# martinber/noaa-apt

Measured on AMD Instinct MI355X. Metric: Msamples/sec WAV->APT-line decode, higher is better.
Workload: dtype f32; 1 GPU; synthetic 48000 Hz APT recording, 600 s (28800000 samples) per GPU, profile=standard: resample 13/50 (959 taps) -> AM envelope -> 37-tap low-pass -> sync correlation + peak picker -> 1198 rows x 2080 px; parallelism=1 GPU(s), 16 independent recordings per GPU and step, no collectives, recordings_per_call=16, mode=strict, rows=1198, n_sync=1199, input_resident_in_hbm=True, distinct_inputs_round_robin=16

## Files before the change

### noaa_apt_amd/csrc/apt_capi.hip

```cpp
#include <cstdio>
#include <cstdlib>
#include <cstring>
#include <memory>
#include <string>

#include "apt_capi_util.hpp"
#include "apt_session.hpp"

namespace {

using namespace apt::capi;

using PlanPtr = std::unique_ptr<aptgpu_plan, apt::capi::PlanDeleter>;


apt::Signal download(const float *d, size_t n, hipStream_t s)
{
    apt::Signal h(n);
    if (n) {
        apt::hip_check(hipMemcpyAsync(h.data(), d, n * sizeof(float), hipMemcpyDeviceToHost, s),
                       "hipMemcpyAsync D2H");
        apt::hip_check(hipStreamSynchronize(s), "hipStreamSynchronize");
    }
    return h;
// ... 66 lines not shown
int aptgpu_plan_get_info(const aptgpu_plan *plan, aptgpu_plan_info *info)
{
    if (!plan || !info) return APTGPU_ERR_INVALID;
    info->l = plan->l;
    info->m = plan->m;
    info->n_resample_taps = static_cast<uint32_t>(plan->taps_resample.size());
    info->n_lowpass_taps = static_cast<uint32_t>(plan->taps_lowpass.size());
    info->n_sync_taps = plan->n_sync_taps;
    info->samples_per_work_row = plan->spr;
    info->min_distance = plan->md;
    info->max_samples = plan->max_samples;
    info->max_work_len = plan->max_work_len;
    info->max_rows = plan->max_rows;
    info->fused = plan->fused;
    info->max_batch = plan->max_batch;
    return APTGPU_OK;
}

int aptgpu_plan_decode_device(aptgpu_plan *plan, int count, const float *const *d_signals,
                              const size_t *n, float *const *d_rows, const size_t *rows_cap,
                              char *err, size_t err_cap)
{
    if (!plan || !d_signals || !n || !d_rows || !rows_cap || count < 0 ||
        count > plan->max_batch) {
        put_err(err, err_cap, "bad argument to aptgpu_plan_decode_device");
        return APTGPU_ERR_INVALID;
    }
    return guarded(err, err_cap, [&] {
        apt::hip_check(hipSetDevice(plan->device), "hipSetDevice");
        for (int i = 0; i < count; ++i)
            if (n[i] > plan->max_samples)
                throw Error{ErrorKind::Invalid, "recording longer than the plan's max_samples"};
        std::vector<aptgpu_plan::Input> ins(static_cast<size_t>(count));
        std::vector<uint64_t> caps(static_cast<size_t>(count));
        for (int i = 0; i < count; ++i) {
            ins[static_cast<size_t>(i)].ptr = d_signals[i];
            ins[static_cast<size_t>(i)].n = n[i];
            caps[static_cast<size_t>(i)] = static_cast<uint64_t>(rows_cap[i]) * 2080u;
        }
        plan->run_call(count, ins.data(), d_rows, caps.data(), false);
        return APTGPU_OK;
    });
}

int aptgpu_plan_synchronize(aptgpu_plan *plan)
{
    if (!plan) return APTGPU_ERR_INVALID;
    (void)hipSetDevice(plan->device);
    try {
        plan->sync_all();
    } catch (const Error &) {
        return APTGPU_ERR_HIP;
    }
    return APTGPU_OK;
}

int aptgpu_plan_join(aptgpu_plan *plan)
{
    if (!plan) return APTGPU_ERR_INVALID;
    if (!plan->user_stream) return aptgpu_plan_synchronize(plan);
    (void)hipSetDevice(plan->device);
    for (hipStream_t st : plan->streams) {
        if (hipEventRecord(plan->ev_user, st) != hipSuccess ||
            hipStreamWaitEvent(plan->user_stream, plan->ev_user, 0) != hipSuccess)
            return APTGPU_ERR_HIP;
    }
    return APTGPU_OK;
}

int aptgpu_plan_results(aptgpu_plan *plan, int count, aptgpu_result *results)
{
    if (!plan || !results || count < 0 || static_cast<size_t>(count) > plan->last_slots.size())
        return APTGPU_ERR_INVALID;
    static_assert(sizeof(aptgpu_result) == sizeof(apt::gpu::Result), "result layout");
    (void)hipSetDevice(plan->device);
    try {
        plan->sync_all();
    } catch (const Error &) {
        return APTGPU_ERR_HIP;
    }
    for (int i = 0; i < count; ++i)
        if (hipMemcpy(results + i, plan->result_of(i), sizeof(aptgpu_result), hipMemcpyDeviceToHost) !=
            hipSuccess)
            return APTGPU_ERR_HIP;
    return APTGPU_OK;
}

int aptgpu_plan_sync_positions(aptgpu_plan *plan, int i, uint64_t *pos, size_t cap, size_t *n_sync)
{
    if (!plan || i < 0 || static_cast<size_t>(i) >= plan->last_slots.size() || !n_sync)
        return APTGPU_ERR_INVALID;
    aptgpu_result r{};
    (void)hipSetDevice(plan->device);
    try {
        plan->sync_all();
    } catch (const Error &) {
        return APTGPU_ERR_HIP;
    }
    if (hipMemcpy(&r, plan->result_of(i), sizeof r, hipMemcpyDeviceToHost) != hipSuccess)
        return APTGPU_ERR_HIP;
    *n_sync = r.n_sync;
    size_t take = r.n_sync < cap ? r.n_sync : cap;
    if (!plan->sync || !pos || take == 0) return APTGPU_OK;
    if (take > plan->slot_of(i).peaks.count) take = plan->slot_of(i).peaks.count;
    std::vector<uint32_t> tmp(take);
    if (hipMemcpy(tmp.data(), plan->slot_of(i).peaks.ptr, take * sizeof(uint32_t),
                  hipMemcpyDeviceToHost) != hipSuccess)
        return APTGPU_ERR_HIP;
    for (size_t k = 0; k < take; ++k) pos[k] = tmp[k];
    return APTGPU_OK;
}

int aptgpu_plan_enable_timing(aptgpu_plan *plan, int on)
{
    if (!plan) return APTGPU_ERR_INVALID;
    plan->timer.enable(on < 0 ? 0 : (on > 2 ? 2 : on));
    return APTGPU_OK;
}

int aptgpu_plan_collect_timing(aptgpu_plan *plan, aptgpu_kernel_time *out, size_t cap, size_t *n_out)
{
    if (!plan || !n_out) return APTGPU_ERR_INVALID;
    try {
        (void)hipSetDevice(plan->device);
        plan->sync_all();
        plan->sync_all();
        auto v = plan->timer.collect(plan->stream);
        *n_out = v.size();
        for (size_t i = 0; i < v.size() && i < cap && out; ++i) out[i] = v[i];
        return APTGPU_OK;
    } catch (const Error &) {
        return APTGPU_ERR_HIP;
    }
}

int aptgpu_plan_read_internal(aptgpu_plan *plan, int i, const char *name, void *host_out,
                              size_t bytes, size_t *size_out)
{
    if (!plan || !name || i < 0 || static_cast<size_t>(i) >= plan->last_slots.size())
        return APTGPU_ERR_INVALID;
    aptgpu_plan::Slot &sl = plan->slot_of(i);
    const void *src = nullptr;
    size_t size = 0;
    const std::string n(name);
    if (n == "inv_sinphi") {
        if (size_out) *size_out = sizeof(float);
        if (host_out && bytes >= sizeof(float)) std::memcpy(host_out, &plan->inv_sinphi, sizeof(float));
        return APTGPU_OK;
    }
    if (n == "filtered") { src = sl.filtered.ptr; size = sl.filtered.count * sizeof(float); }
    else if (n == "correlation") { src = sl.correlation.ptr; size = sl.correlation.count * sizeof(float); }
    else if (n == "group_max") { src = sl.gm.ptr; size = sl.gm.count * sizeof(apt::gpu::GroupMax); }
    else if (n == "terminal_words") { src = sl.words.ptr; size = sl.words.count * sizeof(uint64_t); }
    else if (n == "peaks") { src = sl.peaks.ptr; size = sl.peaks.count * sizeof(uint32_t); }
    else if (n == "picker_flags") { src = sl.flags.ptr; size = sl.flags.count * sizeof(uint32_t); }
    else return APTGPU_ERR_INVALID;
    if (size_out) *size_out = size;
    (void)hipSetDevice(plan->device);
    try {
        plan->sync_all();
    } catch (const Error &) {
        return APTGPU_ERR_HIP;
    }
    const size_t take = bytes < size ? bytes : size;
    if (take && host_out && src &&
        hipMemcpy(host_out, src, take, hipMemcpyDeviceToHost) != hipSuccess)
        return APTGPU_ERR_HIP;
    return APTGPU_OK;
}

}

namespace apt::capi {

int decode_host(const aptgpu_context *ctx_in, const aptgpu_settings *settings, const float *signal,
                const uint8_t *wav_data, const apt::WavInfo *wav, size_t n, uint32_t input_rate_hz, int sync,
                float **rows_out, size_t *n_out, aptgpu_stats *stats, char *err, size_t err_cap)
{
    *rows_out = nullptr;
    *n_out = 0;
    aptgpu_context ctx = ctx_in ? *ctx_in : default_ctx();
    const bool steps = settings->export_wav != 0 && ctx.step != nullptr;

    return guarded(err, err_cap, [&]() -> int {
        const uint32_t work = settings->work_rate;
        if (!wav) step(&ctx, steps, "input", 0, signal, n, input_rate_hz);
        if (!wav || !steps) status(&ctx, 0.1f, "Resampling to " + std::to_string(work));

        const bool cached = !steps && ctx.stream == nullptr;
        SessionLease lease;
        struct PoisonOnThrow {
            SessionLease &l;
            bool ok = false;
            ~PoisonOnThrow() { if (!ok && l) l.poison(); }
        } guard{lease};
        hipStream_t s_for_errors = nullptr;
        auto decode_error = [&](const char *msg) -> Error {
            if (s_for_errors == nullptr || hipStreamSynchronize(s_for_errors) == hipSuccess) guard.ok = true;
            return Error{ErrorKind::Internal, msg};
        };
        PlanPtr own_plan;
        aptgpu_plan *plan = nullptr;
        if (cached) {
            SessionKey key;
            key.device = ctx.device;
            key.mode = ctx.mode;
            key.rate = input_rate_hz;
            key.sync = sync != 0;
            key.per_call = 1;
            key.settings = *settings;
            key.settings.export_wav = 0;
            key.settings.export_resample_filtered = settings->export_resample_filtered ? 1 : 0;
            lease = session_acquire(key, n);
            plan = lease->plan.get();
        } else {
            own_plan.reset(apt::plan_create(&ctx, *settings, input_rate_hz, sync != 0, n, 1,  1));
            plan = own_plan.get();
        }
        if (plan->spr == 0) throw Error{ErrorKind::Invalid, "work_rate too small"};
        hipStream_t s = plan->stream;
        s_for_errors = s;
        const uint64_t w = plan->work_len_for(n);
        const uint64_t out_cap =
            sync ? (plan->spr ? w / plan->spr + 2 : 2) * 2080u : plan->out_len_nosync(w) + 16;

        apt::DeviceBuffer<float> own_in, own_rows;
        apt::DeviceBuffer<uint8_t> own_wav;
        const size_t in_bytes = wav ? wav->data_len : n * sizeof(float);
        void *d_in_ptr = nullptr;
        float *d_rows_ptr = nullptr;
        if (cached) {
            lease->ensure_set(0, in_bytes + 64, out_cap);
            d_in_ptr = lease->sets[0].in[0].ptr;
            d_rows_ptr = lease->sets[0].out[0].ptr;
        } else if (wav) {
            own_wav.alloc(in_bytes + 16);
            d_in_ptr = own_wav.ptr;
        } else {
            own_in.alloc(n + 16);
            d_in_ptr = own_in.ptr;
        }
        if (!cached) {
            own_rows.alloc(out_cap);
            d_rows_ptr = own_rows.ptr;
        }
        struct { float *ptr; } d_rows{d_rows_ptr};
        aptgpu_plan::Input in;
        in.n = n;
        in.ptr = d_in_ptr;
        if (in_bytes)
            apt::hip_check(hipMemcpyAsync(d_in_ptr, wav ? static_cast<const void *>(wav_data) : static_cast<const void *>(signal),
                                          in_bytes, hipMemcpyHostToDevice, s), "hipMemcpyAsync H2D");
        if (wav) {
            in.channels = wav->channels;
            in.bytes_per_sample = wav->bytes_per_sample;
            in.codec = static_cast<int>(wav->codec);
        }

        float *rows_ptr = d_rows.ptr;
        const uint64_t cap64 = out_cap;
        plan->run_call(1, &in, &rows_ptr, &cap64, steps);
        aptgpu_plan::Slot &sl = plan->slot_of(0);
        if (steps) plan->sync_all();
        if (wav && steps) {
            apt::Signal x = download(sl.ingest.ptr, n, s);
            step(&ctx, steps, "input", 0, x.data(), x.size(), input_rate_hz);
            status(&ctx, 0.1f, "Resampling to " + std::to_string(work));
        }

        auto export_expanded = [&](uint64_t cnt, uint32_t rate, auto &&fill) {
            try {
                apt::DeviceBuffer<float> d_ex;
                d_ex.alloc(cnt + 16);
                fill(d_ex.ptr);
                apt::Signal ex = download(d_ex.ptr, cnt, s);
                step(&ctx, steps, "resample_filtered", 0, ex.data(), ex.size(), rate);
                return;
            } catch (const Error &e) {
                if (e.kind != ErrorKind::Hip || e.hip_code != static_cast<int>(hipErrorOutOfMemory)) throw;
                (void)hipGetLastError();
            } catch (const std::bad_alloc &) {
            }
            std::fprintf(stderr, "aptgpu: expanded filtered signal (%llu samples) can't fit in memory, skipping step\n",
                         static_cast<unsigned long long>(cnt));
            step(&ctx, steps, "resample_filtered", 0, nullptr, 0, rate);
        };
        step(&ctx, steps, "resample_filter", 1, plan->taps_resample.data(),
             plan->taps_resample.size(), 0);
        if (w < 10ull * plan->spr) throw decode_error(kTooShort);
        if (steps) {
            if (plan->l > 1 && plan->export_filtered) {
                const uint64_t cnt = apt::fast_resampling_export_geom(n, plan->l, plan->m, plan->taps_resample.size()).expanded;
                export_expanded(cnt, input_rate_hz * plan->l, [&](float *d_ex) {
                    plan->expanded_filtered(s, wav ? sl.ingest.ptr : static_cast<const float *>(d_in_ptr), n, false, d_ex, cnt);
                });
            } else if (plan->l > 1) {
                step(&ctx, steps, "resample_filtered", 0, nullptr, 0, input_rate_hz * plan->l);
            } else {
                apt::DeviceBuffer<float> d_fl;
                d_fl.alloc(n + 16);
                apt::gpu::fir_decimate(s, wav ? sl.ingest.ptr : static_cast<const float *>(d_in_ptr), n, plan->d_taps_resample.ptr,
                                       static_cast<uint32_t>(plan->taps_resample.size()), 1, d_fl.ptr, n);
                apt::Signal fl = download(d_fl.ptr, n, s);
                step(&ctx, steps, "resample_filtered", 0, fl.data(), fl.size(), input_rate_hz);
            }
            apt::Signal r = download(sl.resampled.ptr, w, s);
// ... 361 lines not shown
```

### noaa_apt_amd/csrc/apt_kernels_sync.hip

```cpp
#include "apt_kernels.hpp"
#include "apt_sync_corr.hpp"

#include <hip/hip_runtime.h>

#include <atomic>

#include <cstdlib>
#include <type_traits>

namespace apt::gpu {

namespace {

constexpr int GS = 52;
constexpr uint64_t kGroupMask = (1ull << GS) - 1;
constexpr float kNegInf = -__builtin_huge_valf();

__global__ void __launch_bounds__(256)
k_group_max(const float *__restrict__ corr, uint64_t n_corr, GroupMax *__restrict__ gm, uint32_t ng)
{
    const uint32_t g = blockIdx.x * blockDim.x + threadIdx.x;
    if (g >= ng) return;
    const uint64_t base = static_cast<uint64_t>(g) * GS;
    float mx = kNegInf;
    bool has_nan = false;
    for (int o = 0; o < GS; ++o) {
        const uint64_t i = base + o;
        if (i < n_corr) {
            float v = corr[i];
            if (i == 0 && !(v > 0.f)) v = 0.f;
            mx = fmaxf(mx, v);
            has_nan = has_nan || (v != v);
        }
    }
    gm[g] = has_nan ? GroupMax{-kNegInf, kNegInf} : GroupMax{mx, mx};
}

constexpr int kNodesThreads = 128;
constexpr int kNodesWaves = kNodesThreads / 64;
constexpr int kChunkGroups = 128;
constexpr int kSlotCap = 64;
static_assert(kNodesThreads == kChunkGroups, "one thread per own group");
constexpr uint32_t kNanStartTag = 0x80000000u;
constexpr uint32_t kPosMask = 0x7FFFFFFFu;

__host__ __device__ constexpr uint32_t nodes_window(uint32_t pw) { return (GS + 38u * pw - 1u + 3u) & ~3u; }

__device__ __forceinline__ float wave_prefix_max_dpp(float x)
{
    asm volatile("s_nop 1\n\tv_max_f32_dpp %0, %0, %0 row_shr:1 row_mask:0xf bank_mask:0xf\n\t"
                 "s_nop 1\n\tv_max_f32_dpp %0, %0, %0 row_shr:2 row_mask:0xf bank_mask:0xf\n\t"
                 "s_nop 1\n\tv_max_f32_dpp %0, %0, %0 row_shr:4 row_mask:0xf bank_mask:0xf\n\t"
                 "s_nop 1\n\tv_max_f32_dpp %0, %0, %0 row_shr:8 row_mask:0xf bank_mask:0xf\n\t"
                 "s_nop 1\n\tv_max_f32_dpp %0, %0, %0 row_bcast:15 row_mask:0xa bank_mask:0xf\n\t"
                 "s_nop 1\n\tv_max_f32_dpp %0, %0, %0 row_bcast:31 row_mask:0xc bank_mask:0xf\n\t"
                 "s_nop 1"
                 : "+v"(x));
    return x;
}
__device__ __forceinline__ float wave_suffix_max_excl_dpp(float x, int lane)
{
    float y = -__builtin_huge_valf();
    asm volatile("s_nop 1\n\tv_mov_b32_dpp %0, %1 wave_shl:1 row_mask:0xf bank_mask:0xf\n\t"
                 "s_nop 1\n\tv_max_f32_dpp %0, %0, %0 row_shl:1 row_mask:0xf bank_mask:0xf\n\t"
                 "s_nop 1\n\tv_max_f32_dpp %0, %0, %0 row_shl:2 row_mask:0xf bank_mask:0xf\n\t"
                 "s_nop 1\n\tv_max_f32_dpp %0, %0, %0 row_shl:4 row_mask:0xf bank_mask:0xf\n\t"
                 "s_nop 1\n\tv_max_f32_dpp %0, %0, %0 row_shl:8 row_mask:0xf bank_mask:0xf\n\t"
                 "s_nop 1"
                 : "+v"(y)
                 : "v"(x));
    const float r1 = __builtin_bit_cast(float, __builtin_amdgcn_readlane(__builtin_bit_cast(int, y), 16));
    const float r2 = __builtin_bit_cast(float, __builtin_amdgcn_readlane(__builtin_bit_cast(int, y), 32));
    const float r3 = __builtin_bit_cast(float, __builtin_amdgcn_readlane(__builtin_bit_cast(int, y), 48));
    const float m23 = fmaxf(r2, r3), m123 = fmaxf(r1, m23);
    const float tail = lane < 16 ? m123 : lane < 32 ? m23 : lane < 48 ? r3 : -__builtin_huge_valf();
    return fmaxf(y, tail);
}

__host__ __device__ constexpr uint32_t words_f32_ofs() { return kChunkGroups * 16u; }
__host__ __device__ constexpr uint32_t words_win_ofs(uint32_t r)
{
    return (words_f32_ofs() + (kChunkGroups + r + 1) * 16u + kChunkGroups * 4u + kChunkGroups * 2u + 15u) & ~15u;
}

template <int NL, int PWC>
__device__ __forceinline__ float nodes_eval_window(float *win, bool on, int lane, uint32_t pw, int fast)
{
    constexpr int NLR = NL > 0 ? NL : 1;
    float c = kNegInf;
    if (fast) {
        const uint32_t blen = GS + 36u * pw;
        if constexpr (NL > 0) {
            float bs[NLR];
#pragma unroll
            for (int t = 0; t < NL; ++t) {
                const uint32_t pq = lane + 64u * t;
                bs[t] = pq < blen ? sync_pulse_sum(pw, [&](uint32_t j) { return win[pq + j]; }) : 0.f;
            }
            __builtin_amdgcn_wave_barrier();
#pragma unroll
            for (int t = 0; t < NL; ++t) {
                const uint32_t pq = lane + 64u * t;
                if (pq < blen) win[pq] = bs[t];
            }
            __builtin_amdgcn_wave_barrier();
        } else {
            for (uint32_t p0 = 0; p0 < blen; p0 += 64) {
                const uint32_t pq = p0 + lane;
                const float bs = pq < blen ? sync_pulse_sum(pw, [&](uint32_t j) { return win[pq + j]; }) : 0.f;
                __builtin_amdgcn_wave_barrier();
                if (pq < blen) win[pq] = bs;
                __builtin_amdgcn_wave_barrier();
            }
        }
        if (on) c = sync_corr_from_pulses([&](int k) { return win[lane + k * 2 * pw]; });
    } else {
        if constexpr (PWC >= 4) {
            if (on) c = sync_corr_strict_rolled(pw, [&](uint32_t j) { return win[lane + j]; });
        } else {
            if (on) c = sync_corr_strict(pw, [&](uint32_t j) { return win[lane + j]; });
        }
    }
    return c;
}

template <int NL, int PWC, bool DPP>
__global__ void __launch_bounds__(kNodesThreads, 4)
k_sync_words(const CallArgs call, const SlotPtrs *__restrict__ slots, uint32_t pw_arg, uint32_t r_groups ,
             int fast, int use_corr)
{
    const uint32_t pw = PWC > 0 ? static_cast<uint32_t>(PWC) : pw_arg;
    const RecArgs rec = call.rec[blockIdx.y];
    const uint64_t w = rec.w;
    const uint64_t n_corr = w - 38ull * pw;
    const uint32_t ng = static_cast<uint32_t>((n_corr + GS - 1) / GS);
    if (blockIdx.x * static_cast<uint32_t>(kChunkGroups) >= ng) return;
    const SlotPtrs sp = slots[rec.slot];
    const GroupMax *__restrict__ gm = sp.gm;
    const float *__restrict__ corr = use_corr ? sp.corr : nullptr;
    const float *__restrict__ fsig = sp.f;
    uint32_t *__restrict__ flags = sp.flags;

    extern __shared__ uint64_t lds_nodes[];
    const int R = static_cast<int>(r_groups);
    const int N = kChunkGroups + R + 1;
    uint64_t *s_words = lds_nodes;
    uint64_t *s_nanw = s_words + kChunkGroups;
    float *s_hi = reinterpret_cast<float *>(reinterpret_cast<char *>(lds_nodes) + words_f32_ofs());
    float *s_lo = s_hi + N;
    float *s_ma = s_lo + N;
    float *s_mb = s_ma + N;
    float *s_wm = s_mb + N;
    uint16_t *s_cand = reinterpret_cast<uint16_t *>(s_wm + kChunkGroups);
    const uint32_t wlen = nodes_window(pw);
    float *s_win = reinterpret_cast<float *>(reinterpret_cast<char *>(lds_nodes) + words_win_ofs(r_groups));
    __shared__ uint32_t s_ncand;

    const int tid = threadIdx.x;
    const int lane = tid & 63;
    const int wave = tid >> 6;
    const int64_t g0 = static_cast<int64_t>(blockIdx.x) * kChunkGroups;
    const int64_t gw0 = g0;
    const uint64_t md = static_cast<uint64_t>(R) * GS;

    if (tid == 0) s_ncand = 0;
    if (blockIdx.x == 0 && tid == 0) {
        sp.res->status = -1;
        sp.res->reason = -1;
    }
    for (int q = tid; q < N; q += kNodesThreads) {
        const int64_t g = g0 + q;
        const GroupMax v = g < static_cast<int64_t>(ng) ? gm[g] : GroupMax{kNegInf, kNegInf};
        s_hi[q] = v.hi;
        s_lo[q] = v.lo;
        s_ma[q] = v.lo;
    }
    s_words[tid] = 0ull;
    s_nanw[tid] = 0ull;
    __syncthreads();

    {
        const int W = R - 1;
        float *a = s_ma, *bq = s_mb;
        int K = 1;
        for (; 2 * K <= W; K *= 2) {
            for (int q = tid; q < N; q += kNodesThreads) bq[q] = (q + K < N) ? fmaxf(a[q], a[q + K]) : a[q];
            __syncthreads();
            float *t = a; a = bq; bq = t;
        }
        const int q = tid;
        const int64_t g = g0 + q;
        const float wm = fmaxf(a[q + 1], a[q + 1 + W - K]);
        s_wm[q] = wm;
        if (g < static_cast<int64_t>(ng) && !(wm > s_hi[q])) s_cand[atomicAdd(&s_ncand, 1u)] = static_cast<uint16_t>(q);
        __syncthreads();
    }

    const uint32_t ncand = s_ncand;
    constexpr int kBatch = NL > 0 ? 4 : 1;
    constexpr int NLR = NL > 0 ? NL : 1;
    constexpr uint16_t kDeferred = 0x8000u;
    float *wa = s_win + static_cast<size_t>(wave) * wlen;
    const uint32_t wneed = GS + 38u * pw - 1u;
    auto eval_group = [&](uint64_t base, bool on) -> float {
        for (uint32_t t = lane; t < wlen; t += 64) {
            const uint64_t j = base + t;
            wa[t] = (t < wneed && j < w) ? fsig[j] : 0.f;
        }
        __builtin_amdgcn_wave_barrier();
        const float v = nodes_eval_window<NL, PWC>(wa, on, lane, pw, fast);
        __builtin_amdgcn_wave_barrier();
        return v;
    };
    auto settle = [&](auto exact_tag, int q, float cv, float c2v, bool in_v) -> bool {
        constexpr bool EXACT = decltype(exact_tag)::value;
        const uint64_t base = static_cast<uint64_t>(gw0 + q) * GS;
        const bool in2 = in_v && base + lane + md < n_corr;
        if (in_v && gw0 + q == 0 && lane == 0 && !(cv > 0.f)) cv = 0.f;
        const unsigned long long nanword = __ballot(in_v && cv != cv) & kGroupMask;
        if (cv != cv) cv = kNegInf;
        float sfx_ex;
        if constexpr (DPP) {
            sfx_ex = wave_suffix_max_excl_dpp(cv, lane);
        } else {
            float sfx = cv;
            for (int d = 1; d < 64; d <<= 1) {
                const float o = __shfl_down(sfx, d, 64);
                if (lane + d < 64) sfx = fmaxf(sfx, o);
            }
            sfx_ex = __shfl_down(sfx, 1, 64);
            if (lane == 63) sfx_ex = kNegInf;
        }
        float wm = s_wm[q];
        const bool open_lo = in_v && !(sfx_ex > cv) && !(wm > cv);
        if (__ballot(open_lo) != 0ull) {
            float wm_hi = kNegInf;
            for (int h = q + 1 + lane; h < q + R; h += 64) wm_hi = fmaxf(wm_hi, s_hi[h]);
            for (int d = 32; d >= 1; d >>= 1) wm_hi = fmaxf(wm_hi, __shfl_xor(wm_hi, d, 64));
            const bool open = open_lo && wm_hi > cv;
            if (__ballot(open) != 0ull) {
                if constexpr (!EXACT) {
                    return false;
                } else {
                    float thr = open ? cv : -kNegInf;
                    for (int d = 32; d >= 1; d >>= 1) thr = fminf(thr, __shfl_xor(thr, d, 64));
                    float ex = kNegInf;
#pragma unroll 1
                    for (int h0 = q + 1; h0 < q + R; h0 += 64) {
                        unsigned long long todo = __ballot(h0 + lane < q + R && s_hi[h0 + lane] > thr);
                        while (todo) {
                            const int h = h0 + __ffsll(static_cast<long long>(todo)) - 1;
                            todo &= todo - 1;
                            const int64_t gh = gw0 + h;
                            if (gh >= static_cast<int64_t>(ng)) break;
                            const uint64_t hb = static_cast<uint64_t>(gh) * GS;
                            const bool on = lane < GS && hb + lane < n_corr;
                            float v = kNegInf;
                            if (corr != nullptr) {
                                if (on) v = corr[hb + lane];
                            } else {
                                v = eval_group(hb, on);
                            }
                            if (v != v) v = kNegInf;
                            ex = fmaxf(ex, v);
                        }
                    }
                    for (int d = 32; d >= 1; d >>= 1) ex = fmaxf(ex, __shfl_xor(ex, d, 64));
                    if (open) wm = ex;
                    if (lane == 0) atomicAdd(&flags[7], 1u);
                }
            }
        }
        float wmax = fmaxf(sfx_ex, wm);
        const float gm_ahead = s_hi[q + R];
        if (corr == nullptr && __ballot(in2 && !(wmax > cv) && gm_ahead > cv) != 0ull) c2v = eval_group(base + md, in2);
        if (c2v != c2v) c2v = kNegInf;
        float pfx = c2v;
        if constexpr (DPP) {
            pfx = wave_prefix_max_dpp(pfx);
        } else {
            for (int d = 1; d < 64; d <<= 1) {
                const float o = __shfl_up(pfx, d, 64);
                if (lane >= d) pfx = fmaxf(pfx, o);
            }
        }
        wmax = fmaxf(wmax, pfx);
        const bool term = in_v && !(wmax > cv);
        const unsigned long long word = __ballot(term) & kGroupMask;
        if (lane == 0) {
            s_words[q] = word;
            s_nanw[q] = nanword;
        }
        __builtin_amdgcn_wave_barrier();
        return true;
    };
    bool any_deferred = false;
    for (uint32_t c0 = wave * kBatch; c0 < ncand; c0 += kBatch * kNodesWaves) {
        int qv[kBatch];
        float cv[kBatch], c2v[kBatch];
        bool inv[kBatch];
        float fa[kBatch][NLR];
#pragma unroll
        for (int e = 0; e < kBatch; ++e) {
            const uint32_t ci = c0 + e;
            qv[e] = (ci < ncand) ? s_cand[ci] : -1;
            const int64_t g = gw0 + (qv[e] < 0 ? 0 : qv[e]);
            const uint64_t i = static_cast<uint64_t>(g) * GS + lane;
            inv[e] = qv[e] >= 0 && lane < GS && i < n_corr;
            cv[e] = kNegInf;
            c2v[e] = kNegInf;
            if (corr != nullptr) {
                if (inv[e]) {
                    cv[e] = corr[i];
                    if (i + md < n_corr) c2v[e] = corr[i + md];
                }
            } else if constexpr (NL > 0) {
#pragma unroll
                for (int t = 0; t < NL; ++t) {
                    const uint64_t j = static_cast<uint64_t>(g) * GS + lane + 64u * t;
                    fa[e][t] = (qv[e] >= 0 && lane + 64u * t < wneed && j < w) ? fsig[j] : 0.f;
                }
            }
        }
#pragma unroll
        for (int e = 0; e < kBatch; ++e) {
            if (qv[e] < 0) continue;
            if (corr == nullptr) {
                if constexpr (NL > 0) {
#pragma unroll
                    for (int t = 0; t < NL; ++t)
                        if (lane + 64u * t < wlen) wa[lane + 64 * t] = fa[e][t];
                    __builtin_amdgcn_wave_barrier();
                    cv[e] = nodes_eval_window<NL, PWC>(wa, inv[e], lane, pw, fast);
                    __builtin_amdgcn_wave_barrier();
                } else {
                    cv[e] = eval_group(static_cast<uint64_t>(gw0 + qv[e]) * GS, inv[e]);
                }
            }
            if (!settle(std::false_type{}, qv[e], cv[e], c2v[e], inv[e])) {
                if (lane == 0) s_cand[c0 + e] = static_cast<uint16_t>(qv[e]) | kDeferred;
                any_deferred = true;
            }
        }
    }
    if (any_deferred) {
#pragma unroll 1
        for (uint32_t c0 = wave * kBatch; c0 < ncand; c0 += kBatch * kNodesWaves) {
#pragma unroll 1
            for (uint32_t ci = c0; ci < c0 + kBatch && ci < ncand; ++ci) {
                const uint16_t ent = s_cand[ci];
                if (!(ent & kDeferred)) continue;
                const int q = ent & (kDeferred - 1);
                const uint64_t base = static_cast<uint64_t>(gw0 + q) * GS;
                const bool in_v = lane < GS && base + lane < n_corr;
                float cv = kNegInf, c2v = kNegInf;
                if (corr != nullptr) {
                    if (in_v) {
                        cv = corr[base + lane];
                        if (base + lane + md < n_corr) c2v = corr[base + lane + md];
                    }
                } else {
                    cv = eval_group(base, in_v);
                }
                (void)settle(std::true_type{}, q, cv, c2v, in_v);
            }
        }
    }
    __syncthreads();

    {
        const int64_t g = g0 + tid;
        if (g < static_cast<int64_t>(ng)) {
            sp.words[g] = s_words[tid];
            sp.nanw[g] = s_nanw[tid];
        }
    }
}

__global__ void __launch_bounds__(kNodesThreads)
k_sync_slots(const CallArgs call, const SlotPtrs *__restrict__ slots, uint32_t pw, uint32_t r_groups ,
             uint32_t grid_groups )
{
    const RecArgs rec = call.rec[blockIdx.y];
    const uint64_t n_corr = rec.w - 38ull * pw;
    const uint32_t ng = static_cast<uint32_t>((n_corr + GS - 1) / GS);
    if (blockIdx.x * static_cast<uint32_t>(kChunkGroups) >= ng) return;
    const SlotPtrs sp = slots[rec.slot];
    const uint64_t *__restrict__ words = sp.words;
    const uint64_t *__restrict__ nanw = sp.nanw;
    uint32_t *__restrict__ slot_nt = sp.slot_nt;
    __shared__ uint32_t s_scan[kNodesWaves];
    const int tid = threadIdx.x;
    const int lane = tid & 63;
    const int wave = tid >> 6;
    const int64_t R = r_groups;
    const int64_t g = static_cast<int64_t>(blockIdx.x) * kChunkGroups + tid;
    auto word_at = [&](const uint64_t *p, int64_t gi) -> uint64_t {
        return (gi >= 0 && gi < static_cast<int64_t>(ng)) ? p[gi] : 0ull;
    };
    uint64_t nw = 0, ns = 0;
    if (g < static_cast<int64_t>(ng)) {
        const uint64_t wd = words[g];
        const uint64_t nb = nanw[g];
        const uint64_t prev_bit = word_at(words, g - 1) >> (GS - 1);
        const uint64_t heads = wd & ~(((wd << 1) | prev_bit) & kGroupMask);
        const uint64_t shifted = ((word_at(words, g - R) << 1) | (word_at(words, g - R - 1) >> (GS - 1))) & kGroupMask;
        const uint64_t shifted_nan = ((word_at(nanw, g - R) << 1) | (word_at(nanw, g - R - 1) >> (GS - 1))) & kGroupMask;
        const uint64_t on_grid = (g % grid_groups == 0) ? 1ull : 0ull;
        const uint64_t starts = shifted | shifted_nan | on_grid;
        nw = wd & (heads | starts);
        ns = nb & starts & ~wd;
    }
    const uint32_t cnt = static_cast<uint32_t>(__popcll(nw | ns));
    uint32_t inc = cnt;
    for (int d = 1; d < 64; d <<= 1) {
        const uint32_t o = __shfl_up(inc, d, 64);
        if (lane >= d) inc += o;
    }
    if (lane == 63) s_scan[wave] = inc;
    __syncthreads();
    uint32_t base = 0;
    for (int wv = 0; wv < wave; ++wv) base += s_scan[wv];
    uint32_t total = 0;
    for (int wv = 0; wv < kNodesWaves; ++wv) total += s_scan[wv];
    uint32_t ofs = base + inc - cnt;
    uint64_t bitsleft = nw | ns;
    while (bitsleft) {
        const int bpos = __ffsll(static_cast<long long>(bitsleft)) - 1;
        bitsleft &= bitsleft - 1;
        if (ofs < kSlotCap)
            slot_nt[static_cast<uint64_t>(blockIdx.x) * kSlotCap + ofs] =
                static_cast<uint32_t>(static_cast<uint64_t>(g) * GS + bpos) | (((ns >> bpos) & 1ull) ? kNanStartTag : 0u);
        ++ofs;
    }
    if (tid == 0) {
        sp.slot_cnt[blockIdx.x] = total;
        if (total > kSlotCap) atomicOr(&sp.flags[0], 1u);
    }
}

constexpr int kOrbitThreadsMax = 1024;
constexpr int kMaxLevels = 64;

struct OrbitGeom {
    uint64_t n_corr, work_len;
    uint32_t spr, md;
};

__device__ __forceinline__ uint64_t first_terminal52(const uint64_t *__restrict__ words,
                                                     uint64_t n_groups, uint64_t s)
{
    const int lane = threadIdx.x & 63;
    uint64_t g0 = s / GS;
    const uint32_t sh = static_cast<uint32_t>(s % GS);
    bool first = true;
    while (true) {
        const uint64_t gi = g0 + lane;
        uint64_t word = (gi < n_groups) ? words[gi] : 0ull;
        if (first && lane == 0) word &= (~0ull) << sh;
        const unsigned long long any = __ballot(word != 0ull);
        if (any) {
            const int src = __ffsll(static_cast<long long>(any)) - 1;
            const uint64_t pos = gi * GS + (__ffsll(static_cast<long long>(word)) - 1);
            return __shfl(pos, src, 64);
        }
        first = false;
        g0 += 64;
        if (g0 >= n_groups) return ~0ull;
    }
}

__device__ void orbit_walk52(const uint64_t *__restrict__ words, const uint64_t *__restrict__ nanw,
                             const OrbitGeom &gq, uint32_t *__restrict__ peaks, uint32_t peaks_cap,
                             Result *__restrict__ res)
{
    auto nan_at = [&](uint64_t s) -> bool { return (nanw[s / GS] >> (s % GS)) & 1ull; };
    const int lane = threadIdx.x & 63;
    const uint64_t n_groups = (gq.n_corr + GS - 1) / GS;
    const uint64_t spr = gq.spr, md = gq.md;
    uint64_t len = 1;
    uint64_t u = 0;
    if (gq.n_corr > 0) u = first_terminal52(words, n_groups, 0);
    if (lane == 0 && peaks_cap > 0) peaks[0] = static_cast<uint32_t>(u);
    uint64_t fit = (u + spr < gq.work_len) ? 1 : 0;
    uint64_t last_fit = fit;
    while (gq.n_corr > 0) {
        const uint64_t a = u + md + 1;
        const uint64_t b = (len + 1) * spr;
        const uint64_t s = a > b ? a : b;
        if (s >= gq.n_corr) break;
        const uint64_t c = s / spr;
        for (uint64_t q = len + lane; q + 1 < c; q += 64)
            if (q < peaks_cap) peaks[q] = static_cast<uint32_t>(s);
        if (s + spr < gq.work_len) fit += c - len - 1;
        u = nan_at(s) ? s : first_terminal52(words, n_groups, s);
        if (lane == 0 && c - 1 < peaks_cap) peaks[c - 1] = static_cast<uint32_t>(u);
        last_fit = (u + spr < gq.work_len) ? 1 : 0;
        fit += last_fit;
        len = c;
    }
    if (lane == 0) {
        const bool few = len < 5;
        res->status = few ? 1 : 0;
        res->reason = few ? 2 : 0;
        res->n_sync = static_cast<uint32_t>(len);
        res->n_rows = few ? 0 : static_cast<uint32_t>(fit - last_fit);
        res->work_len = gq.work_len;
        res->n_out = few ? 0 : (fit - last_fit) * 2080u;
    }
}


__device__ __forceinline__ uint32_t gld(const uint32_t *p)
{
    return __hip_atomic_load(p, __ATOMIC_RELAXED, __HIP_MEMORY_SCOPE_AGENT);
}
__device__ __forceinline__ void gst(uint32_t *p, uint32_t v)
{
    __hip_atomic_store(p, v, __ATOMIC_RELAXED, __HIP_MEMORY_SCOPE_AGENT);
}
template <int NT>
__global__ void __launch_bounds__(NT, NT >= 1024 ? 8 : 2)
k_sync_orbit_global(const CallArgs call, const SlotPtrs *__restrict__ slots, uint32_t spr_in, uint32_t md_in,
                    uint32_t pw, int force_walk, uint32_t lds_entries, int alg)
{
    const RecArgs rec = call.rec[blockIdx.x];
    const SlotPtrs sp = slots[rec.slot];
    const uint64_t *__restrict__ words = sp.words;
// ... 512 lines not shown
        if (tid == 0) {
            flags[1] = 1u;
            flags[0] = 0u;
            flags[5] = 0u;
            flags[11] = flags7;
            flags[7] = 0u;
        }
        return;
    }
    if (tid == 0 && !all_done) { gst(w_ja + END, END); gst(w_jb + END, END); gst(w_path, 0u); }
    __syncthreads();

    const uint32_t path_cap = kc + 2;
    const bool direct = !all_done && s_conflict == 0;
    if (direct) {
        const uint32_t endc = s_endcell;
        for (uint32_t k = tid + 1; k < path_cap; k += NT)
            gst(w_path + k, k < endc ? gld(w_succ + k) : END);
        __syncthreads();
    }
    uint32_t *ja = w_ja, *jb = w_jb;
    const uint32_t lds_cap = lds_entries;
    const bool in_lds = !all_done && !direct && path_cap + 2 * (count + 1) <= lds_cap && count < 0xFFFFu;
    if (in_lds) {
        uint16_t *pth = lds_orbit;
        uint16_t *la = pth + path_cap;
        uint16_t *lb = la + (count + 1);
        const uint16_t ENDC = static_cast<uint16_t>(count);
        for (uint32_t idx = tid; idx < count; idx += NT) {
            const uint32_t nx = gld(w_ja + gld(w_list + idx));
            la[idx] = nx == END ? ENDC : static_cast<uint16_t>(nx < base_d ? nx : gld(w_jb + nx));
        }
        if (tid == 0) { la[count] = ENDC; lb[count] = ENDC; pth[0] = 0; }
        __syncthreads();
        for (uint32_t span = 1; span < path_cap; span <<= 1) {
            for (uint32_t mI = tid; mI < span && mI + span < path_cap; mI += NT) pth[mI + span] = la[pth[mI]];
            for (uint32_t idx = tid; idx < count; idx += NT) lb[idx] = la[la[idx]];
            __syncthreads();
            uint16_t *t = la; la = lb; lb = t;
        }
        for (uint32_t k = tid; k < path_cap; k += NT)
            gst(w_path + k, pth[k] == ENDC ? END : gld(w_list + pth[k]));
        __syncthreads();
    }
    if (!all_done && !direct && !in_lds) {
    constexpr int kKeep = 4;
    uint32_t vk[kKeep], jk[kKeep];
#pragma unroll
    for (int j = 0; j < kKeep; ++j) {
        const uint32_t idx = tid + j * NT;
        vk[j] = (idx < count) ? gld(w_list + idx) : END;
    }
#pragma unroll
    for (int j = 0; j < kKeep; ++j) jk[j] = gld(ja + vk[j]);
    for (uint32_t span = 1; span < path_cap; span <<= 1) {
        for (uint32_t mI = tid; mI < span && mI + span < path_cap; mI += NT)
            gst(w_path + mI + span, gld(ja + gld(w_path + mI)));
#pragma unroll
        for (int j = 0; j < kKeep; ++j) jk[j] = gld(ja + jk[j]);
#pragma unroll
        for (int j = 0; j < kKeep; ++j) gst(jb + vk[j], jk[j]);
        for (uint32_t idx = tid + kKeep * NT; idx < count; idx += NT) {
            const uint32_t v = gld(w_list + idx);
            gst(jb + v, gld(ja + gld(ja + v)));
        }
        __syncthreads();
        uint32_t *t = ja; ja = jb; jb = t;
    }
    }
    if (!peaks_done) stamp(1);

    if (!peaks_done) {
    if (tid == 0) { s_plen = 1; s_fit = 0ull; }
    __syncthreads();
    }
    unsigned long long fit_local = 0;
    for (uint32_t k = tid; !peaks_done && k < path_cap; k += NT) {
        const uint32_t v = gld(w_path + k);
        if (v == END) continue;
        uint32_t cell;
        const uint32_t sv = node_start(v, &cell);
        const uint32_t u = gld(w_u + v);
        const bool is_last = (k + 1 >= path_cap) || gld(w_path + k + 1) == END;
        if (k == 0) {
            if (peaks_cap > 0) peaks[0] = u;
            if (!is_last && u + spr < wl32) ++fit_local;
            if (is_last) s_plen = 1;
            continue;
        }
        uint32_t pcell;
        (void)node_start(gld(w_path + k - 1), &pcell);
        const uint32_t c_prev = (k - 1 == 0) ? 1u : pcell;
        const uint32_t c = cell;
        for (uint32_t qv = c_prev; qv + 1 < c; ++qv)
            if (qv < peaks_cap) peaks[qv] = sv;
        if (c - 1 < peaks_cap) peaks[c - 1] = u;
        if (sv + spr < wl32) fit_local += c - c_prev - 1;
        if (!is_last && u + spr < wl32) ++fit_local;
        if (is_last) s_plen = c;
    }
    if (!peaks_done) {
    {
        uint32_t f32v = static_cast<uint32_t>(fit_local);
        for (int d = 32; d >= 1; d >>= 1) f32v += __shfl_down(f32v, d, 64);
        if ((tid & 63) == 0 && f32v) atomicAdd(&s_fit, static_cast<unsigned long long>(f32v));
    }
    __syncthreads();
    }
    if (tid == 0) {
        const uint32_t len = s_plen;
        const bool few = len < 5;
        const uint64_t rows = s_fit;
        res->status = few ? 1 : 0;
        res->reason = few ? 2 : 0;
        res->n_sync = len;
        res->n_rows = few ? 0 : static_cast<uint32_t>(rows);
        res->work_len = gq.work_len;
        res->n_out = few ? 0 : rows * 2080u;
        flags[1] = 2u;
        flags[0] = 0u;
        flags[5] = 0u;
        flags[2] = nt_cap;
        flags[3] = n_nodes;
        flags[4] = all_done ? n_all : count;
        flags[6] = all_done ? 3u : direct ? 1u : (in_lds ? 2u : 0u);
        if (all_done) flags[12] = 0u;
        flags[11] = flags7;
        flags[7] = 0u;
    }
    stamp(2);
}

}

uint32_t sync_group_size() { return GS; }
uint32_t sync_chunk_groups() { return kChunkGroups; }
uint32_t sync_slot_cap() { return kSlotCap; }

void group_max(hipStream_t s, const float *corr, uint64_t n_corr, GroupMax *gm)
{
    const uint32_t ng = static_cast<uint32_t>((n_corr + GS - 1) / GS);
    if (ng == 0) return;
    hipLaunchKernelGGL(k_group_max, dim3((ng + 255) / 256), dim3(256), 0, s, corr, n_corr, gm, ng);
}

void sync_nodes(hipStream_t s, const CallArgs &call, const SlotPtrs *d_slots, uint64_t max_w, uint32_t pw,
                uint32_t spr, uint32_t md, bool fast, bool use_corr, const LaunchSwitches &sw)
{
    if (call.count == 0 || max_w <= 38ull * pw) return;
    const uint64_t n_corr = max_w - 38ull * pw;
    const uint32_t ng = static_cast<uint32_t>((n_corr + GS - 1) / GS);
    const uint32_t chunks = (ng + kChunkGroups - 1) / kChunkGroups;
    const uint32_t r = md / GS;
    const size_t lds = words_win_ofs(r) + static_cast<size_t>(kNodesWaves) * nodes_window(pw) * sizeof(float);
    const dim3 grid(chunks, call.count);
    const uint32_t wneed = GS + 38u * pw - 1u;
    const bool dpp = sw.words_dpp;
#define APT_WORDS_LAUNCH(NL, PWC)                                                                                       \
    do {                                                                                                                \
        if (dpp)                                                                                                        \
            hipLaunchKernelGGL((k_sync_words<NL, PWC, true>), grid, dim3(kNodesThreads), lds, s, call, d_slots, pw, r,  \
                               fast ? 1 : 0, use_corr ? 1 : 0);                                                         \
        else                                                                                                            \
            hipLaunchKernelGGL((k_sync_words<NL, PWC, false>), grid, dim3(kNodesThreads), lds, s, call, d_slots, pw, r, \
                               fast ? 1 : 0, use_corr ? 1 : 0);                                                         \
    } while (0)
    if (pw == 3) APT_WORDS_LAUNCH(3, 3);
    else if (pw == 4) APT_WORDS_LAUNCH(4, 4);
    else if (pw == 5) APT_WORDS_LAUNCH(4, 5);
    else if (wneed <= 192) APT_WORDS_LAUNCH(3, 0);
    else if (wneed <= 256) APT_WORDS_LAUNCH(4, 0);
    else APT_WORDS_LAUNCH(0, 0);
#undef APT_WORDS_LAUNCH
    hipLaunchKernelGGL(k_sync_slots, grid, dim3(kNodesThreads), 0, s, call, d_slots, pw, r, spr / GS);
}

uint32_t sync_nt_cap(uint64_t w)
{
    const uint64_t ng = (w + GS - 1) / GS;
    const uint64_t chunks = (ng + kChunkGroups - 1) / kChunkGroups;
    return static_cast<uint32_t>(chunks * kSlotCap);
}

size_t sync_orbit_ws_words(uint64_t w, uint32_t spr)
{
    const uint64_t nt_cap = sync_nt_cap(w);
    const uint64_t kc = (spr ? w / spr : 0) + 2;
    const uint64_t node_cap = 1 + kc + nt_cap + 1;
    return 4 * node_cap + (node_cap / 32 + 1) + (kc + 2) + (kc + 3) + 64;
}

static bool orbit_all_nodes_available(uint32_t bytes)
{
    constexpr int kMaxDevices = 64;
    static std::atomic<int> state[kMaxDevices];
    int dev = 0;
    (void)hipGetDevice(&dev);
    if (dev < 0 || dev >= kMaxDevices) dev = 0;
    int st = state[dev].load(std::memory_order_acquire);
    if (st == 0) {
        int max_lds = 0;
        const bool ok = hipDeviceGetAttribute(&max_lds, hipDeviceAttributeMaxSharedMemoryPerBlock, dev) == hipSuccess &&
                        max_lds >= static_cast<int>(bytes) &&
                        hipFuncSetAttribute(reinterpret_cast<const void *>(&k_sync_orbit_global<kOrbitThreadsMax>),
                                            hipFuncAttributeMaxDynamicSharedMemorySize, static_cast<int>(bytes)) == hipSuccess;
        (void)hipGetLastError();
        st = ok ? 1 : 2;
        state[dev].store(st, std::memory_order_release);
    }
    return st == 1;
}

void sync_orbit(hipStream_t s, const CallArgs &call, const SlotPtrs *d_slots, uint32_t spr, uint32_t md,
                uint32_t pw, int force, const LaunchSwitches &sw)
{
    if (call.count == 0) return;
    const uint32_t kOrbitLdsEntries = sw.orbit_lds ? 12288u : 0u;
    constexpr uint32_t kAllEntries = 65536u;
    const int alg = (sw.orbit_alg == 0 || kOrbitLdsEntries == 0u || !orbit_all_nodes_available(kAllEntries * sizeof(uint16_t))) ? 0 : 1;
    if (sw.orbit_threads == 256) {
        hipLaunchKernelGGL(k_sync_orbit_global<256>, dim3(call.count), dim3(256), kOrbitLdsEntries * sizeof(uint16_t), s,
                           call, d_slots, spr, md, pw, force == 1 ? 1 : 0, kOrbitLdsEntries, 0);
    } else if (alg == 1) {
        hipLaunchKernelGGL(k_sync_orbit_global<kOrbitThreadsMax>, dim3(call.count), dim3(kOrbitThreadsMax), kAllEntries * sizeof(uint16_t), s,
                           call, d_slots, spr, md, pw, force == 1 ? 1 : 0, kAllEntries, 1);
    } else {
        hipLaunchKernelGGL(k_sync_orbit_global<kOrbitThreadsMax>, dim3(call.count), dim3(kOrbitThreadsMax), kOrbitLdsEntries * sizeof(uint16_t), s,
                           call, d_slots, spr, md, pw, force == 1 ? 1 : 0, kOrbitLdsEntries, 0);
    }
}

}
```

Measured before the change: 547,300 Msamples/s.

## Restructure sync words kernel: 256-group blocks, block-max windows, ballot compaction, direct stores

Rewrites the sync terminal-words kernel to use fixed 256-thread blocks covering 256 groups each. The log-step sliding-window max with repeated barriers is replaced by per-block prefix/suffix max scans plus block totals. The LDS atomic candidate list becomes ballot-based wave compaction, and candidates are interleaved across waves. Words are written straight to global memory instead of being staged in LDS, which shrinks the LDS footprint to raise occupancy, at the cost of more scattered global stores and new scan code that could carry edge-case bugs.

Measured after the change: 553,000 Msamples/s (median of 6 runs). 1.01x the previous value.

```diff
diff --git a/noaa_apt_amd/csrc/apt_capi.hip b/noaa_apt_amd/csrc/apt_capi.hip
--- a/noaa_apt_amd/csrc/apt_capi.hip
+++ b/noaa_apt_amd/csrc/apt_capi.hip
@@ -242,6 +242,7 @@
     else if (n == "correlation") { src = sl.correlation.ptr; size = sl.correlation.count * sizeof(float); }
     else if (n == "group_max") { src = sl.gm.ptr; size = sl.gm.count * sizeof(apt::gpu::GroupMax); }
     else if (n == "terminal_words") { src = sl.words.ptr; size = sl.words.count * sizeof(uint64_t); }
+    else if (n == "nan_words") { src = sl.nanw.ptr; size = sl.nanw.count * sizeof(uint64_t); }
     else if (n == "peaks") { src = sl.peaks.ptr; size = sl.peaks.count * sizeof(uint32_t); }
     else if (n == "picker_flags") { src = sl.flags.ptr; size = sl.flags.count * sizeof(uint32_t); }
     else return APTGPU_ERR_INVALID;
diff --git a/noaa_apt_amd/csrc/apt_kernels_sync.hip b/noaa_apt_amd/csrc/apt_kernels_sync.hip
--- a/noaa_apt_amd/csrc/apt_kernels_sync.hip
+++ b/noaa_apt_amd/csrc/apt_kernels_sync.hip
@@ -77,10 +77,42 @@
     return fmaxf(y, tail);
 }
 
-__host__ __device__ constexpr uint32_t words_f32_ofs() { return kChunkGroups * 16u; }
-__host__ __device__ constexpr uint32_t words_win_ofs(uint32_t r)
-{
-    return (words_f32_ofs() + (kChunkGroups + r + 1) * 16u + kChunkGroups * 4u + kChunkGroups * 2u + 15u) & ~15u;
+constexpr int kWordsThreads = 256;
+constexpr int kWordsWaves = kWordsThreads / 64;
+constexpr int kWordsGroups = 256;
+static_assert(kWordsThreads == kWordsGroups, "one thread per own group");
+__host__ __device__ constexpr uint32_t words_span(uint32_t r) { return kWordsGroups + ((r + 63u) & ~63u); }
+__host__ __device__ constexpr uint32_t words_tot_ofs(uint32_t r) { return 2u * words_span(r) * 4u; }
+__host__ __device__ constexpr uint32_t words_wm_ofs(uint32_t r) { return words_tot_ofs(r) + words_span(r) / 16u * 4u; }
+__host__ __device__ constexpr uint32_t words_cand_ofs(uint32_t r) { return words_wm_ofs(r) + kWordsGroups * 4u; }
+__host__ __device__ constexpr uint32_t words_win_ofs(uint32_t r) { return (words_cand_ofs(r) + kWordsGroups * 2u + 15u) & ~15u; }
+static_assert(words_win_ofs(96) + kWordsWaves * nodes_window(3) * 4u <= 8192u, "pw = 3: 8 KB, what is free beside the front end");
+
+#ifdef APT_WORDS_MARKS
+#define APT_WMARK(name) asm volatile("; APTMARK " name)
+#else
+#define APT_WMARK(name) ((void)0)
+#endif
+
+__device__ __forceinline__ float block_prefix_max(float x, int B, int lane)
+{
+    if (B == 64) return wave_prefix_max_dpp(x);
+    for (int d = 1; d < B; d <<= 1) {
+        const float o = __shfl_up(x, d, 64);
+        if ((lane & (B - 1)) >= d) x = fmaxf(x, o);
+    }
+    return x;
+}
+__device__ __forceinline__ float block_suffix_max_excl(float x, int B, int lane)
+{
+    if (B == 64) return wave_suffix_max_excl_dpp(x, lane);
+    float y = __shfl_down(x, 1, 64);
+    if ((lane & (B - 1)) == B - 1) y = kNegInf;
+    for (int d = 1; d < B; d <<= 1) {
+        const float o = __shfl_down(y, d, 64);
+        if ((lane & (B - 1)) + d < B) y = fmaxf(y, o);
+    }
+    return y;
 }
 
 template <int NL, int PWC>
@@ -125,7 +157,7 @@
 }
 
 template <int NL, int PWC, bool DPP>
-__global__ void __launch_bounds__(kNodesThreads, 4)
+__global__ void __launch_bounds__(kWordsThreads, 4)
 k_sync_words(const CallArgs call, const SlotPtrs *__restrict__ slots, uint32_t pw_arg, uint32_t r_groups ,
              int fast, int use_corr)
 {
@@ -134,86 +166,118 @@
     const uint64_t w = rec.w;
     const uint64_t n_corr = w - 38ull * pw;
     const uint32_t ng = static_cast<uint32_t>((n_corr + GS - 1) / GS);
-    if (blockIdx.x * static_cast<uint32_t>(kChunkGroups) >= ng) return;
+    if (blockIdx.x * static_cast<uint32_t>(kWordsGroups) >= ng) return;
     const SlotPtrs sp = slots[rec.slot];
     const GroupMax *__restrict__ gm = sp.gm;
     const float *__restrict__ corr = use_corr ? sp.corr : nullptr;
     const float *__restrict__ fsig = sp.f;
     uint32_t *__restrict__ flags = sp.flags;
+    uint64_t *__restrict__ words = sp.words;
+    uint64_t *__restrict__ nanw = sp.nanw;
 
     extern __shared__ uint64_t lds_nodes[];
     const int R = static_cast<int>(r_groups);
-    const int N = kChunkGroups + R + 1;
-    uint64_t *s_words = lds_nodes;
-    uint64_t *s_nanw = s_words + kChunkGroups;
-    float *s_hi = reinterpret_cast<float *>(reinterpret_cast<char *>(lds_nodes) + words_f32_ofs());
-    float *s_lo = s_hi + N;
-    float *s_ma = s_lo + N;
-    float *s_mb = s_ma + N;
-    float *s_wm = s_mb + N;
-    uint16_t *s_cand = reinterpret_cast<uint16_t *>(s_wm + kChunkGroups);
+    const int NS = static_cast<int>(words_span(r_groups));
+    char *lds = reinterpret_cast<char *>(lds_nodes);
+    float *s_hi = reinterpret_cast<float *>(lds);
+    float *s_pre = s_hi + NS;
+    float *s_tot = reinterpret_cast<float *>(lds + words_tot_ofs(r_groups));
+    float *s_wm = reinterpret_cast<float *>(lds + words_wm_ofs(r_groups));
+    uint16_t *s_cand = reinterpret_cast<uint16_t *>(lds + words_cand_ofs(r_groups));
     const uint32_t wlen = nodes_window(pw);
-    float *s_win = reinterpret_cast<float *>(reinterpret_cast<char *>(lds_nodes) + words_win_ofs(r_groups));
-    __shared__ uint32_t s_ncand;
+    float *s_win = reinterpret_cast<float *>(lds + words_win_ofs(r_groups));
+    __shared__ uint32_t s_wcnt[kWordsWaves];
 
     const int tid = threadIdx.x;
     const int lane = tid & 63;
     const int wave = tid >> 6;
-    const int64_t g0 = static_cast<int64_t>(blockIdx.x) * kChunkGroups;
+    const int64_t g0 = static_cast<int64_t>(blockIdx.x) * kWordsGroups;
     const int64_t gw0 = g0;
     const uint64_t md = static_cast<uint64_t>(R) * GS;
 
-    if (tid == 0) s_ncand = 0;
     if (blockIdx.x == 0 && tid == 0) {
         sp.res->status = -1;
         sp.res->reason = -1;
     }
-    for (int q = tid; q < N; q += kNodesThreads) {
+
+    APT_WMARK("BEGIN coarse");
+    const int W = R - 1;
+    const int B = W >= 64 ? 64 : W >= 32 ? 32 : 16;
+    float sfx = kNegInf, my_hi = kNegInf;
+    for (int q0 = wave * 64; q0 < NS; q0 += kWordsThreads) {
+        const int q = q0 + lane;
         const int64_t g = g0 + q;
         const GroupMax v = g < static_cast<int64_t>(ng) ? gm[g] : GroupMax{kNegInf, kNegInf};
+        const float lo = v.lo != v.lo ? kNegInf : v.lo;
+        const float pre = block_prefix_max(lo, B, lane);
         s_hi[q] = v.hi;
-        s_lo[q] = v.lo;
-        s_ma[q] = v.lo;
-    }
-    s_words[tid] = 0ull;
-    s_nanw[tid] = 0ull;
+        s_pre[q] = pre;
+        if ((lane & (B - 1)) == B - 1) s_tot[q / B] = pre;
+        if (q0 < kWordsGroups) {
+            sfx = block_suffix_max_excl(lo, B, lane);
+            my_hi = v.hi;
+        }
+    }
     __syncthreads();
-
+    bool is_cand;
     {
-        const int W = R - 1;
-        float *a = s_ma, *bq = s_mb;
-        int K = 1;
-        for (; 2 * K <= W; K *= 2) {
-            for (int q = tid; q < N; q += kNodesThreads) bq[q] = (q + K < N) ? fmaxf(a[q], a[q + K]) : a[q];
-            __syncthreads();
-            float *t = a; a = bq; bq = t;
-        }
         const int q = tid;
+        const int e = q + W;
+        float wm = sfx;
+        for (int b = q / B + 1; b < e / B; ++b) wm = fmaxf(wm, s_tot[b]);
+        wm = fmaxf(wm, s_pre[e]);
+        s_wm[q] = wm;
         const int64_t g = g0 + q;
-        const float wm = fmaxf(a[q + 1], a[q + 1 + W - K]);
-        s_wm[q] = wm;
-        if (g < static_cast<int64_t>(ng) && !(wm > s_hi[q])) s_cand[atomicAdd(&s_ncand, 1u)] = static_cast<uint16_t>(q);
+        is_cand = g < static_cast<int64_t>(ng) && !(wm > my_hi);
+        if (g < static_cast<int64_t>(ng) && !is_cand) {
+            words[g] = 0ull;
+            nanw[g] = 0ull;
+        }
+    }
+    APT_WMARK("END coarse");
+    APT_WMARK("BEGIN compaction");
+    uint32_t ncand;
+    {
+        const unsigned long long bal = __ballot(is_cand);
+        if (lane == 0) s_wcnt[wave] = static_cast<uint32_t>(__popcll(bal));
         __syncthreads();
-    }
-
-    const uint32_t ncand = s_ncand;
+        uint32_t base = 0;
+        ncand = 0;
+        for (int wv = 0; wv < kWordsWaves; ++wv) {
+            const uint32_t c = s_wcnt[wv];
+            base += wv < wave ? c : 0u;
+            ncand += c;
+        }
+        if (is_cand) {
+            const uint32_t below = static_cast<uint32_t>(__popcll(bal & ((1ull << lane) - 1ull)));
+            s_cand[base + below] = static_cast<uint16_t>(tid);
+        }
+        __syncthreads();
+    }
+    APT_WMARK("END compaction");
+
     constexpr int kBatch = NL > 0 ? 4 : 1;
     constexpr int NLR = NL > 0 ? NL : 1;
     constexpr uint16_t kDeferred = 0x8000u;
     float *wa = s_win + static_cast<size_t>(wave) * wlen;
     const uint32_t wneed = GS + 38u * pw - 1u;
     auto eval_group = [&](uint64_t base, bool on) -> float {
+        APT_WMARK("BEGIN window_loads");
         for (uint32_t t = lane; t < wlen; t += 64) {
             const uint64_t j = base + t;
             wa[t] = (t < wneed && j < w) ? fsig[j] : 0.f;
         }
         __builtin_amdgcn_wave_barrier();
+        APT_WMARK("END window_loads");
+        APT_WMARK("BEGIN chains");
         const float v = nodes_eval_window<NL, PWC>(wa, on, lane, pw, fast);
         __builtin_amdgcn_wave_barrier();
+        APT_WMARK("END chains");
         return v;
     };
     auto settle = [&](auto exact_tag, int q, float cv, float c2v, bool in_v) -> bool {
         constexpr bool EXACT = decltype(exact_tag)::value;
+        APT_WMARK("BEGIN settle");
         const uint64_t base = static_cast<uint64_t>(gw0 + q) * GS;
         const bool in2 = in_v && base + lane + md < n_corr;
         if (in_v && gw0 + q == 0 && lane == 0 && !(cv > 0.f)) cv = 0.f;
@@ -240,6 +304,7 @@
             const bool open = open_lo && wm_hi > cv;
             if (__ballot(open) != 0ull) {
                 if constexpr (!EXACT) {
+                    APT_WMARK("END settle");
                     return false;
                 } else {
                     float thr = open ? cv : -kNegInf;
@@ -273,7 +338,11 @@
         }
         float wmax = fmaxf(sfx_ex, wm);
         const float gm_ahead = s_hi[q + R];
+        APT_WMARK("END settle");
+        APT_WMARK("BEGIN md_ahead");
         if (corr == nullptr && __ballot(in2 && !(wmax > cv) && gm_ahead > cv) != 0ull) c2v = eval_group(base + md, in2);
+        APT_WMARK("END md_ahead");
+        APT_WMARK("BEGIN settle");
         if (c2v != c2v) c2v = kNegInf;
         float pfx = c2v;
         if constexpr (DPP) {
@@ -287,22 +356,24 @@
         wmax = fmaxf(wmax, pfx);
         const bool term = in_v && !(wmax > cv);
         const unsigned long long word = __ballot(term) & kGroupMask;
+        APT_WMARK("END settle");
+        APT_WMARK("BEGIN word_stores");
         if (lane == 0) {
-            s_words[q] = word;
-            s_nanw[q] = nanword;
-        }
-        __builtin_amdgcn_wave_barrier();
+            words[gw0 + q] = word;
+            nanw[gw0 + q] = nanword;
+        }
+        APT_WMARK("END word_stores");
         return true;
     };
     bool any_deferred = false;
-    for (uint32_t c0 = wave * kBatch; c0 < ncand; c0 += kBatch * kNodesWaves) {
+    for (uint32_t c0 = wave; c0 < ncand; c0 += kBatch * kWordsWaves) {
         int qv[kBatch];
         float cv[kBatch], c2v[kBatch];
         bool inv[kBatch];
         float fa[kBatch][NLR];
 #pragma unroll
         for (int e = 0; e < kBatch; ++e) {
-            const uint32_t ci = c0 + e;
+            const uint32_t ci = c0 + e * kWordsWaves;
             qv[e] = (ci < ncand) ? s_cand[ci] : -1;
             const int64_t g = gw0 + (qv[e] < 0 ? 0 : qv[e]);
             const uint64_t i = static_cast<uint64_t>(g) * GS + lane;
@@ -315,11 +386,13 @@
                     if (i + md < n_corr) c2v[e] = corr[i + md];
                 }
             } else if constexpr (NL > 0) {
+                APT_WMARK("BEGIN window_loads");
 #pragma unroll
                 for (int t = 0; t < NL; ++t) {
                     const uint64_t j = static_cast<uint64_t>(g) * GS + lane + 64u * t;
                     fa[e][t] = (qv[e] >= 0 && lane + 64u * t < wneed && j < w) ? fsig[j] : 0.f;
                 }
+                APT_WMARK("END window_loads");
             }
         }
 #pragma unroll
@@ -331,23 +404,26 @@
                     for (int t = 0; t < NL; ++t)
                         if (lane + 64u * t < wlen) wa[lane + 64 * t] = fa[e][t];
                     __builtin_amdgcn_wave_barrier();
+                    APT_WMARK("BEGIN chains");
                     cv[e] = nodes_eval_window<NL, PWC>(wa, inv[e], lane, pw, fast);
                     __builtin_amdgcn_wave_barrier();
+                    APT_WMARK("END chains");
                 } else {
                     cv[e] = eval_group(static_cast<uint64_t>(gw0 + qv[e]) * GS, inv[e]);
                 }
             }
             if (!settle(std::false_type{}, qv[e], cv[e], c2v[e], inv[e])) {
-                if (lane == 0) s_cand[c0 + e] = static_cast<uint16_t>(qv[e]) | kDeferred;
+                if (lane == 0) s_cand[c0 + e * kWordsWaves] = static_cast<uint16_t>(qv[e]) | kDeferred;
                 any_deferred = true;
             }
         }
     }
     if (any_deferred) {
+        APT_WMARK("BEGIN deferred");
 #pragma unroll 1
-        for (uint32_t c0 = wave * kBatch; c0 < ncand; c0 += kBatch * kNodesWaves) {
+        for (uint32_t c0 = wave; c0 < ncand; c0 += kBatch * kWordsWaves) {
 #pragma unroll 1
-            for (uint32_t ci = c0; ci < c0 + kBatch && ci < ncand; ++ci) {
+            for (uint32_t ci = c0; ci < c0 + kBatch * kWordsWaves && ci < ncand; ci += kWordsWaves) {
                 const uint16_t ent = s_cand[ci];
                 if (!(ent & kDeferred)) continue;
                 const int q = ent & (kDeferred - 1);
@@ -365,15 +441,7 @@
                 (void)settle(std::true_type{}, q, cv, c2v, in_v);
             }
         }
-    }
-    __syncthreads();
-
-    {
-        const int64_t g = g0 + tid;
-        if (g < static_cast<int64_t>(ng)) {
-            sp.words[g] = s_words[tid];
-            sp.nanw[g] = s_nanw[tid];
-        }
+        APT_WMARK("END deferred");
     }
 }
 
@@ -1192,17 +1260,18 @@
     const uint32_t ng = static_cast<uint32_t>((n_corr + GS - 1) / GS);
     const uint32_t chunks = (ng + kChunkGroups - 1) / kChunkGroups;
     const uint32_t r = md / GS;
-    const size_t lds = words_win_ofs(r) + static_cast<size_t>(kNodesWaves) * nodes_window(pw) * sizeof(float);
+    const size_t lds = words_win_ofs(r) + static_cast<size_t>(kWordsWaves) * nodes_window(pw) * sizeof(float);
+    const dim3 grid_w((ng + kWordsGroups - 1) / kWordsGroups, call.count);
     const dim3 grid(chunks, call.count);
     const uint32_t wneed = GS + 38u * pw - 1u;
     const bool dpp = sw.words_dpp;
 #define APT_WORDS_LAUNCH(NL, PWC)                                                                                       \
     do {                                                                                                                \
         if (dpp)                                                                                                        \
-            hipLaunchKernelGGL((k_sync_words<NL, PWC, true>), grid, dim3(kNodesThreads), lds, s, call, d_slots, pw, r,  \
+            hipLaunchKernelGGL((k_sync_words<NL, PWC, true>), grid_w, dim3(kWordsThreads), lds, s, call, d_slots, pw, r,  \
                                fast ? 1 : 0, use_corr ? 1 : 0);                                                         \
         else                                                                                                            \
-            hipLaunchKernelGGL((k_sync_words<NL, PWC, false>), grid, dim3(kNodesThreads), lds, s, call, d_slots, pw, r, \
+            hipLaunchKernelGGL((k_sync_words<NL, PWC, false>), grid_w, dim3(kWordsThreads), lds, s, call, d_slots, pw, r, \
                                fast ? 1 : 0, use_corr ? 1 : 0);                                                         \
     } while (0)
     if (pw == 3) APT_WORDS_LAUNCH(3, 3);
```
